# weihaoysgs/ssvio

Hardware: AMD Instinct MI355X
Metric: stereo frames/s (ORB extract + row-band match + triangulate + one local BA per frame) on 1241x376 (higher is better)
Workload: dtype u8 (front-end) + f64 (BA)

## Files before the change

### include/ssx_test_hooks.h

```cpp
#ifndef SSX_TEST_HOOKS_H
#define SSX_TEST_HOOKS_H
#include "ssx.h"

#ifdef __cplusplus
extern "C" {
#endif

SSX_API int32_t ssx_ba_window_selftest(uint32_t seed, int32_t steps);

SSX_API int64_t ssx_debug_kernel_dynamic_lds(const char* kernel);
SSX_API void ssx_debug_set_dense_slabs(int32_t mode);

SSX_API void ssx_debug_set_trial_finish(int32_t mode);

SSX_API double ssx_ba_debug_prepare_seconds(const ssx_ba_problem* prob, int32_t reps);

SSX_API int32_t ssx_ba_debug_upload_format(const ssx_ba_problem* prob);

SSX_API uint64_t ssx_ba_debug_prepare_digest(const ssx_ba_problem* prob, int32_t threads);


SSX_API ssx_status ssx_ba_linearize(ssx_ctx* ctx, const ssx_ba_problem* prob, double huber_delta, int32_t jac_mode,
                            double* Hpp, double* bp, double* Hll, double* bl, double* Hpl, double* err,
                            double* chi2);

SSX_API ssx_status ssx_orb_stage_level(ssx_ctx* ctx, int32_t image, int32_t level, int32_t blurred,
                                       uint8_t* out, int32_t out_cap, int32_t* rows, int32_t* cols);
SSX_API ssx_status ssx_orb_stage_candidates(ssx_ctx* ctx, int32_t image, int32_t level, int32_t cap,
                                            ssx_keypoint* out, int32_t* n);

SSX_API ssx_status ssx_lk_stage_level(ssx_ctx* ctx, int32_t which, int32_t level, uint8_t* out, int32_t out_cap,
                                      int32_t* rows, int32_t* cols);
SSX_API ssx_status ssx_lk_stage_deriv(ssx_ctx* ctx, int32_t level, int16_t* out, int32_t out_cap, int32_t* rows,
                                      int32_t* cols);

#ifdef __cplusplus
}
#endif
#endif
```

### ssvio_amd/csrc/octree.hip

```cpp
#include "orb_ws.hpp"

namespace ssxorb {

namespace {

typedef unsigned long long u64;
constexpr int T = OCT_THREADS;
constexpr int NW = T / 64;
constexpr unsigned NONE = 0xFFFFu;
struct Box { int16_t ulx, uly, brx, bry; };

struct Tab {
  u64* c4;
  u64* kid4;
  Box* box;
  uint32_t* key;
  uint16_t* cnt;
  uint16_t* pidx;
  uint16_t* newpos;
  uint16_t* proc;
  uint16_t* exp;
};

__device__ __forceinline__ Tab carve(uint8_t* base, int LN)
{
  Tab o;
  const size_t n = (size_t)LN;
  o.c4 = (u64*)base;
  o.kid4 = o.c4 + n;
  o.box = (Box*)(o.kid4 + n);
  o.key = (uint32_t*)(o.box + 2 * n);
  o.cnt = (uint16_t*)(o.key + n);
  o.pidx = o.cnt + 2 * n;
  o.newpos = o.pidx + n;
  o.proc = o.newpos + n;
  o.exp = o.proc + n;
  return o;
}
static_assert(OCT_NODE_BYTES == 8 + 8 + 16 + 4 + 4 + 2 + 2 + 2 + 4, "Tab layout and OCT_NODE_BYTES disagree");

__device__ __forceinline__ u64 block_scan(u64 v, u64 (*s_w)[NW], int& par, u64& total)
{
  const int lane = threadIdx.x & 63, wave = threadIdx.x >> 6;
  u64 inc = v;
#pragma unroll
  for (int o = 1; o < 64; o <<= 1) {
    const u64 up = __shfl_up(inc, o);
    if (lane >= o) inc += up;
  }
  if (lane == 63) s_w[par][wave] = inc;
  __syncthreads();
  u64 before = 0, tot = 0;
#pragma unroll
  for (int w = 0; w < NW; ++w) {
    const u64 x = s_w[par][w];
    tot += x;
    if (w < wave) before += x;
  }
  par ^= 1;
  total = tot;
  return before + (inc - v);
}

__device__ __forceinline__ int quadrant(int x, int y, const Box& n)
{
  const int mx = n.ulx + ((n.brx - n.ulx + 1) >> 1);
  const int my = n.uly + ((n.bry - n.uly + 1) >> 1);
  return (x < mx) ? ((y < my) ? 0 : 2) : ((y < my) ? 1 : 3);
}

__device__ __forceinline__ unsigned f16(u64 v, int q) { return (unsigned)((v >> (16 * q)) & 0xFFFFu); }
__device__ __forceinline__ int pk_x(uint32_t p) { return (int)(p & 0xFFF); }
__device__ __forceinline__ int pk_y(uint32_t p) { return (int)((p >> 12) & 0xFFF); }
__device__ __forceinline__ uint32_t pk_r(uint32_t p) { return p >> 24; }
__device__ __forceinline__ int nonzero4(u64 c) { return (f16(c, 0) > 0) + (f16(c, 1) > 0) + (f16(c, 2) > 0) + (f16(c, 3) > 0); }
__device__ __forceinline__ int above1_4(u64 c) { return (f16(c, 0) > 1) + (f16(c, 1) > 1) + (f16(c, 2) > 1) + (f16(c, 3) > 1); }

template <bool GLOBAL_TAB, bool GLOBAL_KEYS>
__global__ __launch_bounds__(OCT_THREADS) void k_octree(OrbDev d)
{
  extern __shared__ __attribute__((aligned(16))) uint8_t smem[];
  __shared__ u64 s_w[2][NW];
  __shared__ int s_root[64], s_rootpos[64];
  __shared__ int s_i[2];
  const int img = blockIdx.x, level = blockIdx.y, t = threadIdx.x;
  const int lane = t & 63;
  if (d.detect_only && level > 0) return;
  const int il = img * d.nlevels + level;
  const int LN = d.oct_ln;
  Tab tb;
  uint32_t* s_cellpos;
  const int CAP = d.oct_cand_cap;
  uint8_t* scratch = d.oct + (size_t)il * d.oct_stride;
  if constexpr (GLOBAL_TAB) {
    tb = carve(scratch + (GLOBAL_KEYS ? 6 * (size_t)CAP : 0), LN);
    s_cellpos = reinterpret_cast<uint32_t*>(smem);
  } else {
    tb = carve(smem, LN);
    s_cellpos = reinterpret_cast<uint32_t*>(smem + (((size_t)OCT_NODE_BYTES * LN + 15) & ~size_t(15)));
  }
  uint32_t* s_kpk;
  uint16_t* s_kn;
  if constexpr (GLOBAL_KEYS) {
    s_kpk = reinterpret_cast<uint32_t*>(scratch);
    s_kn = reinterpret_cast<uint16_t*>(s_kpk + CAP);
  } else {
    s_kpk = s_cellpos + ((d.oct_max_cells + 1 + 3) & ~3);
    s_kn = reinterpret_cast<uint16_t*>(s_kpk + CAP);
  }
  const int N = d.feat[level];
  const int cell0 = d.lvl_cell0[level], cell1 = d.lvl_cell0[level + 1];
  const int ncell = cell1 - cell0;
  const int* ccount = d.cell_count + (size_t)img * d.n_cells + cell0;
  const uint32_t* __restrict__ ccand = d.cell_cand + ((size_t)img * d.n_cells + cell0) * CELL_CAP;
  int par = 0;

  int M;
  {
    const int chunk = (ncell + T - 1) / T;
    const int lo = min(t * chunk, ncell), hi = min(lo + chunk, ncell);
    u64 mine = 0;
    for (int c = lo; c < hi; ++c) mine += (u64)ccount[c];
    u64 total;
    uint32_t pos = (uint32_t)block_scan(mine, s_w, par, total);
    for (int c = lo; c < hi; ++c) { s_cellpos[c] = pos; pos += (uint32_t)ccount[c]; }
    if (t == 0) {
      s_cellpos[ncell] = (uint32_t)total;
      d.lvl_ncand[il] = (int)total;
      if (total > (u64)CAP) atomicOr(&d.status[img], 1);
    }
    M = (int)min(total, (u64)CAP);
    if (t < 64) s_root[t] = 0;
  }
  __syncthreads();
  int* sel_count = d.sel_count + il;
  uint32_t* sel = d.sel + (size_t)il * SEL_CAP;
  if (M == 0) { if (t == 0) *sel_count = 0; return; }

  const int minX = EDGE_THRESHOLD - 3, minY = minX;
  const int maxX = d.lvl_cols[level] - EDGE_THRESHOLD + 3, maxY = d.lvl_rows[level] - EDGE_THRESHOLD + 3;
  const int nIni = (int)roundf((float)(maxX - minX) / (float)(maxY - minY));
  if (nIni < 1 || nIni > 64) { if (t == 0) *sel_count = 0; return; }
  const float hX = (float)(maxX - minX) / (float)nIni;
  const int kchunk = (M + T - 1) / T;
  const int p0 = min(t * kchunk, M);
  const int nk = min(kchunk, M - p0);
  {
    int c = 0, off = 0, cend = 0;
    if (nk > 0) {
      int lo = 0, hi = ncell;
      while (hi - lo > 1) { const int mid = (lo + hi) >> 1; if (s_cellpos[mid] <= (uint32_t)p0) lo = mid; else hi = mid; }
      c = lo;
      off = p0 - (int)s_cellpos[c];
      cend = (int)(s_cellpos[c + 1] - s_cellpos[c]);
    }
    int run_root = -1, run_n = 0;
    for (int k = 0; k < nk; ++k) {
      while (off >= cend) { ++c; off = 0; cend = (int)(s_cellpos[c + 1] - s_cellpos[c]); }
      const uint32_t v = ccand[(size_t)c * CELL_CAP + off];
      ++off;
      s_kpk[k * T + t] = v;
      const int rt = (int)((float)pk_x(v) / hX);
      const int root = rt >= nIni ? nIni - 1 : rt;
      s_kn[k * T + t] = (uint16_t)root;
      if (root != run_root) {
        if (run_n > 0) atomicAdd(&s_root[run_root], run_n);
        run_root = root; run_n = 0;
      }
      ++run_n;
    }
    if (run_n > 0) atomicAdd(&s_root[run_root], run_n);
  }
  __syncthreads();
  if (t < 64) {
    const int c = t < nIni ? s_root[t] : 0;
    const u64 bal = __ballot(c > 0);
    const int pos = __popcll(bal & ((1ull << lane) - 1ull));
    s_rootpos[t] = pos;
    if (c > 0) {
      Box b;
      b.ulx = (int16_t)(int)(hX * (float)t); b.uly = 0;
      b.brx = (int16_t)(int)(hX * (float)(t + 1)); b.bry = (int16_t)(maxY - minY);
      tb.box[pos] = b;
      tb.cnt[pos] = (uint16_t)c;
    }
    if (t == 0) s_i[0] = __popcll(bal);
  }
  __syncthreads();
  int nNodes = s_i[0];
  for (int k = 0; k < nk; ++k) s_kn[k * T + t] = (uint16_t)s_rootpos[s_kn[k * T + t]];

  int cur = 0, ecur = 0, nExp = 0, phase = 1, guard = 0;
  bool finish = false;
  while (!finish && ++guard < 256) {
    const Box* bx = tb.box + cur * LN;
    const uint16_t* ct = tb.cnt + cur * LN;
    Box* nbx = tb.box + (cur ^ 1) * LN;
    uint16_t* nct = tb.cnt + (cur ^ 1) * LN;
    const uint16_t* exp_cur = tb.exp + ecur * LN;
    uint16_t* exp_nxt = tb.exp + (ecur ^ 1) * LN;
    const int prevSize = nNodes;
    const int nchunk = (nNodes + T - 1) / T;
    const int nlo = min(t * nchunk, nNodes), nhi = min(nlo + nchunk, nNodes);
    int m = 0;
    if (phase == 1) {
      u64 mine = 0;
      for (int j = nlo; j < nhi; ++j) mine += ct[j] > 1;
      u64 total;
      uint32_t pos = (uint32_t)block_scan(mine, s_w, par, total);
      for (int j = nlo; j < nhi; ++j) {
        if (ct[j] > 1) { tb.proc[pos] = (uint16_t)j; tb.pidx[j] = (uint16_t)pos; tb.c4[pos] = 0; ++pos; }
// ... 81 lines not shown
    for (int i = plo; i < phi; ++i) {
      const int j = tb.proc[i];
      const Box x = bx[j];
      const u64 c = tb.c4[i];
      const int cc = nonzero4(c);
      const int mx = x.ulx + ((x.brx - x.ulx + 1) >> 1);
      const int my = x.uly + ((x.bry - x.uly + 1) >> 1);
      const int first = (int)Tchild - (int)run_cc - cc;
      int above = cc;
      u64 kid = 0;
      for (int q = 0; q < 4; ++q) {
        const int n = (int)f16(c, q);
        if (n == 0) continue;
        --above;
        const int id = first + above;
        Box ch;
        ch.ulx = (int16_t)((q & 1) ? mx : x.ulx); ch.brx = (int16_t)((q & 1) ? x.brx : mx);
        ch.uly = (int16_t)((q & 2) ? my : x.uly); ch.bry = (int16_t)((q & 2) ? x.bry : my);
        nbx[id] = ch;
        nct[id] = (uint16_t)n;
        kid |= (u64)id << (16 * q);
        if (n > 1) exp_nxt[run_ex++] = (uint16_t)id;
      }
      tb.kid4[i] = kid;
      run_cc += (uint32_t)cc;
    }
    for (int j = nlo; j < nhi; ++j)
      if (tb.pidx[j] == NONE) {
        const uint32_t np = Tchild + run_k++;
        tb.newpos[j] = (uint16_t)np;
        nbx[np] = bx[j];
        nct[np] = ct[j];
      }
    __syncthreads();
    for (int k = 0; k < nk; ++k) {
      const int kn = s_kn[k * T + t];
      const int j = kn & 0x3FFF, q = kn >> 14;
      const unsigned pi = tb.pidx[j];
      s_kn[k * T + t] = (pi != NONE) ? (uint16_t)f16(tb.kid4[pi], q) : tb.newpos[j];
    }
    __syncthreads();
    cur ^= 1;
    ecur ^= 1;
    nNodes = nNew;
    nExp = (int)EXtot;
    if (nNodes >= N || nNodes == prevSize) finish = true;
    else if (phase == 1 && nNodes + 3 * nExp > N) phase = 2;
  }
  __syncthreads();
  {
    uint32_t* best = tb.key;
    for (int j = t; j < nNodes; j += T) best[j] = 0;
    __syncthreads();
    {
      int run_j = -1;
      uint32_t run_best = 0;
      for (int k = 0; k < nk; ++k) {
        const int j = s_kn[k * T + t] & 0x3FFF;
        const uint32_t v = (pk_r(s_kpk[k * T + t]) << 16) | (uint32_t)(0xFFFF - (p0 + k));
        if (j != run_j) {
          if (run_j >= 0) atomicMax(&best[run_j], run_best);
          run_j = j; run_best = 0;
        }
        run_best = max(run_best, v);
      }
      if (run_j >= 0) atomicMax(&best[run_j], run_best);
    }
    __syncthreads();
    const int nOut = min(nNodes, SEL_CAP);
    for (int k = 0; k < nk; ++k) {
      const int j = s_kn[k * T + t] & 0x3FFF;
      const uint32_t c = s_kpk[k * T + t];
      if (j < nOut && best[j] == ((pk_r(c) << 16) | (uint32_t)(0xFFFF - (p0 + k)))) sel[j] = c;
    }
    if (t == 0) {
      *sel_count = nOut;
      if (nNodes > SEL_CAP) atomicOr(&d.status[img], 4);
    }
  }
}

}

void launch_octree(const OrbDev& o, hipStream_t s)
{
  const dim3 grid(o.I, o.detect_only ? 1 : o.nlevels);
  const size_t tab = o.oct_global_tab ? 0 : (((size_t)OCT_NODE_BYTES * o.oct_ln + 15) & ~size_t(15));
  const size_t lds = tab + 4 * (size_t)((o.oct_max_cells + 1 + 3) & ~3) + (o.oct_global_keys ? 0 : 6 * (size_t)o.oct_cand_cap);
  void (*kern)(OrbDev) = o.oct_global_tab ? (o.oct_global_keys ? k_octree<true, true> : k_octree<true, false>)
                                          : (o.oct_global_keys ? k_octree<false, true> : k_octree<false, false>);
  if (lds > 48 * 1024)
    (void)hipFuncSetAttribute(reinterpret_cast<const void*>(kern), hipFuncAttributeMaxDynamicSharedMemorySize, (int)lds);
  hipLaunchKernelGGL(kern, grid, dim3(OCT_THREADS), lds, s, o);
}

}
```

### ssvio_amd/csrc/orb.hip

```cpp
#include <algorithm>
#include <cfloat>
#include <cmath>
#include <vector>

#include "ctx.hpp"
#include "orb_ws.hpp"
#include "../../include/ssx_test_hooks.h"

namespace ssxorb {

__constant__ __attribute__((aligned(16))) int8_t c_pattern[256 * 4] = {
#include "brief_pattern.inc"
};
__constant__ int c_umax[16] = {15, 15, 15, 15, 14, 14, 14, 13, 13, 12, 11, 10, 9, 8, 6, 3};
__constant__ int c_gauss[7] = {18, 34, 49, 55, 49, 34, 18};
__constant__ int c_ring_dx[16] = {0, 1, 2, 3, 3, 3, 2, 1, 0, -1, -2, -3, -3, -3, -2, -1};
__constant__ int c_ring_dy[16] = {3, 3, 2, 1, 0, -1, -2, -3, -3, -3, -2, -1, 0, 1, 2, 3};

struct ResizeQuad {
  uint32_t s0;
  uint32_t sel0, sel1;
  uint32_t pad;
  uint32_t w[4];
};

constexpr int RS_ROWS = 4;
constexpr int RS_LOOP = 4;
template <bool WIDE8>
__global__ __launch_bounds__(256) void k_resize(const uint8_t* __restrict__ src_base, uint8_t* __restrict__ dst_base,
                                                size_t img_stride_bytes, int spitch, int drows, int dcols, int dpitch,
                                                const ResizeQuad* __restrict__ xtab, const uint2* __restrict__ ytab, int loops)
{
  const int q = blockIdx.x * 64 + threadIdx.x;
  if (4 * q >= dcols) return;
  const uint8_t* src = src_base + (size_t)blockIdx.z * img_stride_bytes;
  uint8_t* dst = dst_base + (size_t)blockIdx.z * img_stride_bytes;
  const uint4 ta = reinterpret_cast<const uint4*>(xtab)[2 * q], tw = reinterpret_cast<const uint4*>(xtab)[2 * q + 1];
#pragma unroll 1
  for (int it = 0; it < loops; ++it) {
  const int dy0 = ((blockIdx.y * loops + it) * 4 + __builtin_amdgcn_readfirstlane(threadIdx.y)) * RS_ROWS;
  if (dy0 >= drows) break;
  uint32_t p00[RS_ROWS], p01[RS_ROWS], p10[RS_ROWS], p11[RS_ROWS];
  int b0[RS_ROWS], b1[RS_ROWS];
  uint2 w0[RS_ROWS], w1[RS_ROWS];
#pragma unroll
  for (int r = 0; r < RS_ROWS; ++r) {
    const uint2 yt = ytab[min(dy0 + r, drows - 1)];
    b0[r] = (int)(yt.y & 0xFFFFu); b1[r] = (int)(yt.y >> 16);
    const uint8_t* r0 = src + (size_t)(yt.x & 0xFFFFu) * spitch + ta.x;
    const uint8_t* r1 = src + (size_t)(yt.x >> 16) * spitch + ta.x;
    if (WIDE8) {
      __builtin_memcpy(&w0[r], r0, 8);
      __builtin_memcpy(&w1[r], r1, 8);
    } else {
      p00[r] = p01[r] = p10[r] = p11[r] = 0;
#pragma unroll
      for (int k = 0; k < 4; ++k) {
        const int o0 = (ta.y >> (8 * k)) & 0xFF, o1 = (ta.z >> (8 * k)) & 0xFF;
        p00[r] |= (uint32_t)r0[o0] << (8 * k); p01[r] |= (uint32_t)r0[o1] << (8 * k);
        p10[r] |= (uint32_t)r1[o0] << (8 * k); p11[r] |= (uint32_t)r1[o1] << (8 * k);
      }
    }
  }
  const uint32_t wa[4] = {tw.x, tw.y, tw.z, tw.w};
#pragma unroll
  for (int r = 0; r < RS_ROWS; ++r) {
    if (WIDE8) {
      p00[r] = __builtin_amdgcn_perm(w0[r].y, w0[r].x, ta.y); p01[r] = __builtin_amdgcn_perm(w0[r].y, w0[r].x, ta.z);
      p10[r] = __builtin_amdgcn_perm(w1[r].y, w1[r].x, ta.y); p11[r] = __builtin_amdgcn_perm(w1[r].y, w1[r].x, ta.z);
    }
    uint32_t out = 0;
#pragma unroll
    for (int k = 0; k < 4; ++k) {
      const int a0 = (int)(wa[k] & 0xFFFFu), a1 = (int)(wa[k] >> 16);
      const int S0 = (int)((p00[r] >> (8 * k)) & 0xFF) * a0 + (int)((p01[r] >> (8 * k)) & 0xFF) * a1;
      const int S1 = (int)((p10[r] >> (8 * k)) & 0xFF) * a0 + (int)((p11[r] >> (8 * k)) & 0xFF) * a1;
      const uint32_t v = (uint32_t)((((b0[r] * (S0 >> 4)) >> 16) + ((b1[r] * (S1 >> 4)) >> 16) + 2) >> 2);
      out |= (v & 0xFFu) << (8 * k);
    }
    if (dy0 + r < drows) *reinterpret_cast<uint32_t*>(dst + (size_t)(dy0 + r) * dpitch + 4 * q) = out;
  }
  }
}
// ... 836 lines not shown
    for (int j = 0; j < nCols; ++j) {
      const float iniX = (float)(minBorderX + j * wCell);
      float maxX = iniX + wCell + 6;
      if (iniX >= maxBorderX - 6) continue;
      if (maxX > maxBorderX) maxX = (float)maxBorderX;
      Cell c;
      c.x0 = (int16_t)(int)iniX; c.y0 = (int16_t)(int)iniY;
      c.w = (int16_t)((int)maxX - (int)iniX); c.h = (int16_t)((int)maxY - (int)iniY);
      c.ox = (int16_t)(j * wCell); c.oy = (int16_t)(i * hCell);
      c.level = (int16_t)level; c.pad = 0;
      out.push_back(c);
    }
  }
}

}

ssx_status plan(ssx_ctx* ctx, int rows, int cols, int I, const ssx_orb_params& prm, bool has_mask, bool detect_only)
{
  OrbWorkspace* ws = get_ws(ctx);
  const int nlevels = detect_only ? 1 : prm.nlevels;
  if (rows <= 2 * EDGE_THRESHOLD || cols <= 2 * EDGE_THRESHOLD || rows > 4000 || cols > 4000) {
    ctx->set_error("ssx_orb: image %dx%d outside the supported range (40..4000 per side)", cols, rows);
    return SSX_ERR_INVALID_ARG;
  }
  if (nlevels < 1 || nlevels > MAX_LEVELS || !(prm.scale_factor > 1.0f) || prm.nfeatures < 1 || prm.nfeatures > SEL_CAP - 8 || I < 1) {
    ctx->set_error("ssx_orb: unsupported parameters (nlevels=%d scale=%g nfeatures=%d)", prm.nlevels, (double)prm.scale_factor, prm.nfeatures);
    return SSX_ERR_INVALID_ARG;
  }
  if (ws->planned && ws->rows == rows && ws->cols == cols && ws->I == I && ws->nlevels == nlevels &&
      ws->nfeatures == prm.nfeatures && ws->ini_th == prm.ini_th_fast && ws->min_th == prm.min_th_fast &&
      ws->has_mask == (int)has_mask && ws->detect_only == (int)detect_only && ws->scale_factor == prm.scale_factor)
    return SSX_OK;
  SSX_HIP_TRY(ctx, hipSetDevice(ctx->device));
  SSX_HIP_TRY(ctx, hipStreamSynchronize(ctx->stream));
  OrbDev d{};
  d.I = I; d.nlevels = nlevels; d.ini_th = prm.ini_th_fast; d.min_th = prm.min_th_fast;
  d.has_mask = has_mask; d.detect_only = detect_only;
  float scale[MAX_LEVELS], inv[MAX_LEVELS];
  scale[0] = 1.0f;
  for (int i = 1; i < nlevels; ++i) scale[i] = scale[i - 1] * prm.scale_factor;
  for (int i = 0; i < nlevels; ++i) inv[i] = 1.0f / scale[i];
  if (detect_only) {
    d.feat[0] = prm.nfeatures;
  } else {
    const float factor = 1.0f / prm.scale_factor;
    float nDesired = prm.nfeatures * (1 - factor) / (1 - (float)std::pow((double)factor, (double)nlevels));
    int sum = 0;
    for (int l = 0; l < nlevels - 1; ++l) {
      d.feat[l] = h_round(nDesired);
      sum += d.feat[l];
      nDesired *= factor;
    }
    d.feat[nlevels - 1] = std::max(prm.nfeatures - sum, 0);
  }
  std::vector<Cell> cells;
  size_t off = 0;
  int out_cap = 32;
  for (int l = 0; l < nlevels; ++l) {
    d.scale[l] = scale[l];
    d.lvl_cols[l] = h_round((float)cols * inv[l]);
    d.lvl_rows[l] = h_round((float)rows * inv[l]);
    d.lvl_pitch[l] = (d.lvl_cols[l] + 127) & ~127;
    d.lvl_off[l] = off;
    off += (size_t)d.lvl_pitch[l] * d.lvl_rows[l];
    d.lvl_cell0[l] = (int)cells.size();
    make_cells(d.lvl_rows[l], d.lvl_cols[l], l, cells);
    {
      const int bw = d.lvl_cols[l] - 2 * (EDGE_THRESHOLD - 3), bh = d.lvl_rows[l] - 2 * (EDGE_THRESHOLD - 3);
      const int n_ini = bh > 0 ? (int)std::lround((double)bw / (double)bh) : 0;
      out_cap += std::max(d.feat[l] + 4, 4 * std::max(n_ini, 0) + 4);
    }
    if (d.feat[l] + 8 > SEL_CAP) {
      ctx->set_error("ssx_orb: %d features on level %d exceed the octree node capacity", d.feat[l], l);
      return SSX_ERR_UNSUPPORTED;
    }
  }
  d.lvl_cell0[nlevels] = (int)cells.size();
  for (int l = nlevels + 1; l <= MAX_LEVELS; ++l) d.lvl_cell0[l] = (int)cells.size();
  d.n_cells = (int)cells.size();
  d.pyr_bytes = (off + 255) & ~size_t(255);
  d.out_cap = out_cap;
  {
    int maxN = 256;
    for (int l = 0; l < (detect_only ? 1 : nlevels); ++l) maxN = std::max(maxN, d.feat[l]);
    d.oct_ln = (maxN + 8 + 7) & ~7;
    d.oct_max_cells = 1;
    for (int l = 0; l < nlevels; ++l) d.oct_max_cells = std::max(d.oct_max_cells, d.lvl_cell0[l + 1] - d.lvl_cell0[l]);
    d.oct_global_keys = (size_t)d.lvl_rows[0] * d.lvl_cols[0] > 600000;
    d.oct_cand_cap = d.oct_global_keys ? CAND_CAP_BIG : CAND_CAP;
    const size_t key_lds = d.oct_global_keys ? 0 : 6 * (size_t)CAND_CAP;
    if (4 * (size_t)(d.oct_max_cells + 8) + key_lds > (size_t)OCT_LDS_BUDGET) {
      ctx->set_error("ssx_orb: %d grid cells on one level exceed the octree workgroup's LDS", d.oct_max_cells);
      return SSX_ERR_UNSUPPORTED;
    }
    d.oct_global_tab = (size_t)OCT_NODE_BYTES * d.oct_ln + 4 * (size_t)(d.oct_max_cells + 8) + key_lds > (size_t)OCT_LDS_BUDGET;
    d.oct_stride = ((d.oct_global_keys ? 6 * (size_t)CAND_CAP_BIG : 0) + (d.oct_global_tab ? (size_t)OCT_NODE_BYTES * d.oct_ln : 0) + 255) & ~size_t(255);
    if (!d.oct_global_keys && !d.oct_global_tab) d.oct_stride = 0;
  }
  {
    int tile = 16, npx = 1, t0 = 0;
    for (const Cell& c : cells) {
      const int tw = ((c.x0 & 3) + c.w + 3) & ~3;
      tile = std::max(tile, tw * (int)c.h);
      npx = std::max(npx, std::max(c.w - 6, 0) * std::max(c.h - 6, 0));
    }
    d.fast_tile_bytes = (tile + 15) & ~15;
    d.fast_lds_per_wave = 2 * d.fast_tile_bytes + ((2 * npx + 15) & ~15);
    d.gauss_run = I > 8 ? GT_RUN : 1;
    for (int l = 0; l < nlevels; ++l) {
      d.gauss_tile0[l] = t0;
      t0 += ((((d.lvl_cols[l] + GT_W - 1) / GT_W) + d.gauss_run - 1) / d.gauss_run) * ((d.lvl_rows[l] + GT_H - 1) / GT_H);
    }
    for (int l = nlevels; l <= MAX_LEVELS; ++l) d.gauss_tile0[l] = t0;
  }
  std::vector<ResizeQuad> xtab;
  std::vector<uint2> ytab;
  for (int l = 1; l < nlevels; ++l) {
    const int scols = d.lvl_cols[l - 1], srows = d.lvl_rows[l - 1], dcols = d.lvl_cols[l], drows = d.lvl_rows[l];
    const double scale_x = 1. / ((double)dcols / scols), scale_y = 1. / ((double)drows / srows);
    d.rs_xoff[l] = (int)xtab.size();
    d.rs_yoff[l] = (int)ytab.size();
    d.rs_wide8[l] = 1;
    for (int q = 0; 4 * q < dcols; ++q) {
      ResizeQuad rq{};
      for (int k = 0; k < 4 && 4 * q + k < dcols; ++k) {
        const int dx = 4 * q + k;
        float fx = (float)((dx + 0.5) * scale_x - 0.5);
        int sx = (int)std::floor(fx);
        fx -= sx;
        if (sx < 0) { fx = 0; sx = 0; }
        if (sx >= scols - 1) { fx = 0; sx = scols - 1; }
        const int a0 = h_round((1.f - fx) * 2048), a1 = h_round(fx * 2048);
        const int sx1 = std::min(sx + 1, scols - 1);
        if (k == 0) rq.s0 = (uint32_t)sx;
        const int o0 = sx - (int)rq.s0, o1 = sx1 - (int)rq.s0;
        if (o1 > 7) d.rs_wide8[l] = 0;
        if (o1 > 255) {
          ctx->set_error("ssx_orb: pyramid scale factor %g is too large for the resize tables", (double)prm.scale_factor);
          return SSX_ERR_UNSUPPORTED;
        }
        rq.sel0 |= (uint32_t)o0 << (8 * k);
        rq.sel1 |= (uint32_t)o1 << (8 * k);
        rq.w[k] = (uint32_t)a0 | ((uint32_t)a1 << 16);
      }
      xtab.push_back(rq);
    }
    for (int dy = 0; dy < drows; ++dy) {
      float fy = (float)((dy + 0.5) * scale_y - 0.5);
      const int sy = (int)std::floor(fy);
      fy -= sy;
      const int b0 = h_round((1.f - fy) * 2048), b1 = h_round(fy * 2048);
      const int sy0 = std::min(std::max(sy, 0), srows - 1), sy1 = std::min(std::max(sy + 1, 0), srows - 1);
      ytab.push_back(make_uint2((uint32_t)sy0 | ((uint32_t)sy1 << 16), (uint32_t)b0 | ((uint32_t)b1 << 16)));
    }
  }
  for (const Cell& c : cells)
    if (c.w > ROI_MAX || c.h > ROI_MAX) {
      ctx->set_error("ssx_orb: grid cell %dx%d exceeds the %d-px LDS tile", c.w, c.h, ROI_MAX);
      return SSX_ERR_UNSUPPORTED;
    }
  Layout lay;
  const size_t o_cells = lay.take(sizeof(Cell) * std::max<size_t>(cells.size(), 1));
  const size_t o_xtab = lay.take(sizeof(ResizeQuad) * std::max<size_t>(xtab.size(), 1));
  const size_t o_ytab = lay.take(sizeof(uint2) * std::max<size_t>(ytab.size(), 4));
  const size_t o_pyr = lay.take(d.pyr_bytes * I);
  const size_t o_mask = lay.take(has_mask ? d.pyr_bytes * I : 256);
  const size_t o_blur = lay.take(d.pyr_bytes * I);
  const size_t o_ccount = lay.take(sizeof(int) * (size_t)I * std::max(d.n_cells, 1));
  const size_t o_ccand = lay.take(sizeof(uint32_t) * (size_t)I * std::max(d.n_cells, 1) * CELL_CAP);
  const size_t o_oct = lay.take(std::max<size_t>(d.oct_stride * (size_t)I * nlevels, 256));
  const size_t o_ncand = lay.take(sizeof(int) * (size_t)I * nlevels);
  const size_t o_selc = lay.take(sizeof(int) * (size_t)I * nlevels);
  const size_t o_sel = lay.take(sizeof(uint32_t) * (size_t)I * nlevels * SEL_CAP);
  const size_t o_ang = lay.take(sizeof(float) * (size_t)I * nlevels * SEL_CAP);
  const size_t o_status = lay.take(sizeof(int) * (size_t)I);
  const size_t o_kps = lay.take(sizeof(ssx_keypoint) * (size_t)I * out_cap);
  const size_t o_desc = lay.take((size_t)32 * I * out_cap);
  const size_t o_n = lay.take(sizeof(int) * (size_t)I);
  SSX_HIP_TRY(ctx, ws->arena.reserve(lay.off));
  char* base = ws->arena.as<char>();
  d.cells = (const Cell*)(base + o_cells);
  d.rs_xtab = (const ResizeQuad*)(base + o_xtab);
  d.rs_ytab = (const uint2*)(base + o_ytab);
  d.pyr = (uint8_t*)(base + o_pyr);
  d.maskpyr = (uint8_t*)(base + o_mask);
  d.blur = (uint8_t*)(base + o_blur);
  d.cell_count = (int*)(base + o_ccount);
  d.cell_cand = (uint32_t*)(base + o_ccand);
  d.oct = (uint8_t*)(base + o_oct);
  d.lvl_ncand = (int*)(base + o_ncand);
  d.sel_count = (int*)(base + o_selc);
  d.sel = (uint32_t*)(base + o_sel);
  d.sel_angle = (float*)(base + o_ang);
  d.status = (int*)(base + o_status);
  d.out_kps = (uint8_t*)(base + o_kps);
  d.out_desc = (uint8_t*)(base + o_desc);
  d.out_n = (int*)(base + o_n);
  if (!cells.empty())
    SSX_HIP_TRY(ctx, hipMemcpyAsync(base + o_cells, cells.data(), sizeof(Cell) * cells.size(), hipMemcpyHostToDevice, ctx->stream));
  if (!xtab.empty()) {
    SSX_HIP_TRY(ctx, hipMemcpyAsync(base + o_xtab, xtab.data(), sizeof(ResizeQuad) * xtab.size(), hipMemcpyHostToDevice, ctx->stream));
    SSX_HIP_TRY(ctx, hipMemcpyAsync(base + o_ytab, ytab.data(), sizeof(uint2) * ytab.size(), hipMemcpyHostToDevice, ctx->stream));
  }
  SSX_HIP_TRY(ctx, hipStreamSynchronize(ctx->stream));
  ws->dev = d;
  ws->rows = rows; ws->cols = cols; ws->I = I; ws->nlevels = nlevels; ws->nfeatures = prm.nfeatures;
  ws->ini_th = prm.ini_th_fast; ws->min_th = prm.min_th_fast; ws->has_mask = has_mask; ws->detect_only = detect_only;
  ws->scale_factor = prm.scale_factor;
  ws->planned = true;
  return SSX_OK;
}

static void launch_pyramid(ssx_ctx* ctx, const OrbDev& d, hipStream_t s, int images)
{
  for (int l = 1; l < d.nlevels; ++l) {
    if (d.lvl_cols[l] <= 0 || d.lvl_rows[l] <= 0) break;
    const int loops = images > 8 ? RS_LOOP : 1;
    const dim3 grid((d.lvl_cols[l] + 255) / 256, (d.lvl_rows[l] + 4 * RS_ROWS * loops - 1) / (4 * RS_ROWS * loops), images);
    auto kern = d.rs_wide8[l] ? k_resize<true> : k_resize<false>;
    for (int m = 0; m < (d.has_mask ? 2 : 1); ++m) {
      uint8_t* pyr = m ? d.maskpyr : d.pyr;
      SSX_PROF(ctx, KID_ORB_RESIZE, hipLaunchKernelGGL(kern, grid, dim3(64, 4), 0, s, pyr + d.lvl_off[l - 1], pyr + d.lvl_off[l], d.pyr_bytes,
                         d.lvl_pitch[l - 1], d.lvl_rows[l], d.lvl_cols[l], d.lvl_pitch[l], d.rs_xtab + d.rs_xoff[l], d.rs_ytab + d.rs_yoff[l], loops));
    }
  }
}

ssx_status stage_level0(ssx_ctx* ctx, const uint8_t* imgs_dev, int stride, size_t img_bytes, const uint8_t* masks_dev,
                        int mask_stride, size_t mask_bytes)
{
  OrbWorkspace* ws = get_ws(ctx);
  const OrbDev& d = ws->dev;
  const dim3 grid((d.lvl_cols[0] + 511) / 512, (d.lvl_rows[0] + 3) / 4, d.I);
  SSX_PROF(ctx, KID_ORB_MISC, hipLaunchKernelGGL(k_copy_level0, grid, dim3(64, 4), 0, ctx->stream, imgs_dev, stride, img_bytes, d.pyr, d.pyr_bytes,
                     d.lvl_rows[0], d.lvl_cols[0], d.lvl_pitch[0]));
  if (d.has_mask)
    SSX_PROF(ctx, KID_ORB_MISC, hipLaunchKernelGGL(k_copy_level0, grid, dim3(64, 4), 0, ctx->stream, masks_dev, mask_stride, mask_bytes, d.maskpyr,
                       d.pyr_bytes, d.lvl_rows[0], d.lvl_cols[0], d.lvl_pitch[0]));
  SSX_HIP_TRY(ctx, hipGetLastError());
  return SSX_OK;
}

ssx_status run_pipeline(ssx_ctx* ctx)
{
  OrbWorkspace* ws = get_ws(ctx);
  const OrbDev& d = ws->dev;
  hipStream_t s = ctx->stream;
  SSX_HIP_TRY(ctx, hipMemsetAsync(d.status, 0, sizeof(int) * d.I, s));
  constexpr int FAST_WPW = 2;
  if (FAST_WPW * (size_t)d.fast_lds_per_wave > 48 * 1024)
    (void)hipFuncSetAttribute(reinterpret_cast<const void*>(k_fast_cells), hipFuncAttributeMaxDynamicSharedMemorySize,
                              (int)(FAST_WPW * (size_t)d.fast_lds_per_wave));
  auto launch_fast = [&](hipStream_t st, int c0, int c1) {
    if (c1 > c0)
      SSX_PROF_ON(ctx, st, KID_ORB_FAST, hipLaunchKernelGGL(k_fast_cells, dim3((c1 - c0 + FAST_WPW - 1) / FAST_WPW, d.I), dim3(64 * FAST_WPW),
                                                            FAST_WPW * (size_t)d.fast_lds_per_wave, st, d, c0, c1));
  };
  static const bool no_fork_env = getenv("SSX_ORB_NO_FORK") != nullptr;
  const bool fork = !d.detect_only && ctx->aux != nullptr && d.I > 2 && !no_fork_env;
  if (fork) {
    SSX_HIP_TRY(ctx, hipEventRecord(ctx->ev_fork, s));
    SSX_HIP_TRY(ctx, hipStreamWaitEvent(ctx->aux, ctx->ev_fork, 0));
    launch_fast(ctx->aux, 0, d.lvl_cell0[1]);
    SSX_HIP_TRY(ctx, hipEventRecord(ctx->ev_fast0, ctx->aux));
    launch_pyramid(ctx, d, s, d.I);
    SSX_HIP_TRY(ctx, hipEventRecord(ctx->ev_pyr, s));
    SSX_HIP_TRY(ctx, hipStreamWaitEvent(ctx->aux, ctx->ev_pyr, 0));
    SSX_PROF_ON(ctx, ctx->aux, KID_ORB_GAUSS, hipLaunchKernelGGL(k_gauss7, dim3(d.gauss_tile0[d.nlevels], d.I), dim3(256), 0, ctx->aux, d));
    SSX_HIP_TRY(ctx, hipEventRecord(ctx->ev_join, ctx->aux));
    launch_fast(s, d.lvl_cell0[1], d.n_cells);
    SSX_HIP_TRY(ctx, hipStreamWaitEvent(s, ctx->ev_fast0, 0));
  } else {
    launch_pyramid(ctx, d, s, d.I);
    if (!d.detect_only)
      SSX_PROF(ctx, KID_ORB_GAUSS, hipLaunchKernelGGL(k_gauss7, dim3(d.gauss_tile0[d.nlevels], d.I), dim3(256), 0, s, d));
    launch_fast(s, 0, d.n_cells);
  }
  SSX_PROF(ctx, KID_ORB_OCTREE, launch_octree(d, s));
  if (d.detect_only) {
    SSX_PROF(ctx, KID_ORB_MISC, hipLaunchKernelGGL(k_finalize_detect, dim3((SEL_CAP + 255) / 256, d.I), dim3(256), 0, s, d));
  } else {
    const dim3 kgrid((d.out_cap + 4 + 4 * OB_KPW - 1) / (4 * OB_KPW), d.I);
    if (fork) SSX_HIP_TRY(ctx, hipStreamWaitEvent(s, ctx->ev_join, 0));
    SSX_PROF(ctx, KID_ORB_BRIEF, hipLaunchKernelGGL(k_orient_brief, kgrid, dim3(256), 0, s, d));
  }
  SSX_PROF(ctx, KID_ORB_MISC, hipLaunchKernelGGL(k_counts, dim3((d.I + 63) / 64), dim3(64), 0, s, d));
  SSX_HIP_TRY(ctx, hipGetLastError());
  return SSX_OK;
}

namespace {

ssx_status run_host_image(ssx_ctx* ctx, const uint8_t* img, int stride, int rows, int cols, const uint8_t* mask,
                          int mask_stride, const ssx_orb_params& prm, bool detect_only)
{
  ssx_status st = plan(ctx, rows, cols, 1, prm, mask != nullptr, detect_only);
  if (st != SSX_OK) return st;
  OrbWorkspace* ws = get_ws(ctx);
  const size_t bytes = (size_t)rows * cols;
  SSX_HIP_TRY(ctx, ws->input.reserve(2 * bytes + 512));
  SSX_HIP_TRY(ctx, ws->stage.reserve(2 * bytes + 512));
  uint8_t* hs = ws->stage.as<uint8_t>();
  for (int y = 0; y < rows; ++y) memcpy(hs + (size_t)y * cols, img + (size_t)y * stride, cols);
  if (mask)
    for (int y = 0; y < rows; ++y) memcpy(hs + bytes + (size_t)y * cols, mask + (size_t)y * mask_stride, cols);
  SSX_HIP_TRY(ctx, hipMemcpyAsync(ws->input.p, hs, mask ? 2 * bytes : bytes, hipMemcpyHostToDevice, ctx->stream));
  st = stage_level0(ctx, ws->input.as<uint8_t>(), cols, bytes, ws->input.as<uint8_t>() + bytes, cols, bytes);
  if (st != SSX_OK) return st;
  return run_pipeline(ctx);
}

ssx_status fetch_image_result(ssx_ctx* ctx, int image, int cap, ssx_keypoint* kps_out, uint8_t* desc_out, int32_t* n)
{
  OrbWorkspace* ws = get_ws(ctx);
  const OrbDev& d = ws->dev;
  int hn[2] = {0, 0};
  SSX_HIP_TRY(ctx, hipMemcpyAsync(&hn[0], d.out_n + image, sizeof(int), hipMemcpyDeviceToHost, ctx->stream));
  SSX_HIP_TRY(ctx, hipMemcpyAsync(&hn[1], d.status + image, sizeof(int), hipMemcpyDeviceToHost, ctx->stream));
  SSX_HIP_TRY(ctx, hipStreamSynchronize(ctx->stream));
  if (hn[1] != 0) {
    ctx->set_error("ssx_orb: internal capacity exceeded (status bits %d: 1=candidates 2=octree nodes 4=outputs)", hn[1]);
    return SSX_ERR_CAPACITY;
  }
  *n = hn[0];
  if (hn[0] > cap) {
    ctx->set_error("ssx_orb: %d keypoints but capacity %d", hn[0], cap);
    return SSX_ERR_CAPACITY;
  }
  if (hn[0] > 0) {
    if (kps_out)
      SSX_HIP_TRY(ctx, hipMemcpyAsync(kps_out, d.out_kps + (size_t)image * d.out_cap * sizeof(ssx_keypoint),
                                      sizeof(ssx_keypoint) * hn[0], hipMemcpyDeviceToHost, ctx->stream));
    if (desc_out && !d.detect_only)
      SSX_HIP_TRY(ctx, hipMemcpyAsync(desc_out, d.out_desc + (size_t)image * d.out_cap * 32, (size_t)32 * hn[0],
                                      hipMemcpyDeviceToHost, ctx->stream));
    SSX_HIP_TRY(ctx, hipStreamSynchronize(ctx->stream));
  }
  return SSX_OK;
}

}

ssx_status fetch_image(ssx_ctx* ctx, int image, int cap, ssx_keypoint* kps_out, uint8_t* desc_out, int32_t* n)
{
  return fetch_image_result(ctx, image, cap, kps_out, desc_out, n);
}

}

using namespace ssxorb;

extern "C" {

void ssx_orb_default_params(ssx_orb_params* p)
{
  if (!p) return;
  p->nfeatures = 2000; p->scale_factor = 1.2f; p->nlevels = 8; p->ini_th_fast = 20; p->min_th_fast = 7;
}

ssx_status ssx_orb_detect(ssx_ctx* ctx, const uint8_t* img, int32_t stride, int32_t rows, int32_t cols,
                          const uint8_t* mask, int32_t mask_stride, const ssx_orb_params* prm, int32_t cap,
// ... 183 lines not shown
  const size_t o_desc = lay.take((size_t)32 * n_in);
  const size_t o_keep = lay.take((size_t)n_in);
  SSX_HIP_TRY(ctx, ws->input.reserve(lay.off));
  SSX_HIP_TRY(ctx, ws->stage.reserve(lay.off));
  char* hs = ws->stage.as<char>();
  for (int y = 0; y < rows; ++y) memcpy(hs + o_img + (size_t)y * cols, img + (size_t)y * stride, cols);
  memcpy(hs + o_in, kps_in, sizeof(ssx_keypoint) * n_in);
  char* base = ws->input.as<char>();
  SSX_HIP_TRY(ctx, hipMemcpyAsync(base, hs, in_bytes, hipMemcpyHostToDevice, ctx->stream));
  st = stage_level0(ctx, (const uint8_t*)(base + o_img), cols, bytes, nullptr, 0, 0);
  if (st != SSX_OK) return st;
  hipStream_t s = ctx->stream;
  launch_pyramid(ctx, d, s, 1);
  SSX_PROF(ctx, KID_ORB_GAUSS, hipLaunchKernelGGL(k_gauss7, dim3(d.gauss_tile0[d.nlevels], 1), dim3(256), 0, s, d));
  DescribeAt a;
  a.in = (const ssx_keypoint*)(base + o_in); a.out = (ssx_keypoint*)(base + o_out); a.desc = (uint8_t*)(base + o_desc);
  a.keep = (uint8_t*)(base + o_keep); a.n_in = n_in;
  SSX_PROF(ctx, KID_ORB_BRIEF, hipLaunchKernelGGL(k_describe_at, dim3((n_in + 3) / 4), dim3(256), 0, s, d, a));
  SSX_HIP_TRY(ctx, hipGetLastError());
  SSX_HIP_TRY(ctx, hipMemcpyAsync(hs + o_out, base + o_out, lay.off - o_out, hipMemcpyDeviceToHost, s));
  SSX_HIP_TRY(ctx, hipStreamSynchronize(s));
  const ssx_keypoint* ok = (const ssx_keypoint*)(hs + o_out);
  const uint8_t* od = (const uint8_t*)(hs + o_desc);
  const uint8_t* keep = (const uint8_t*)(hs + o_keep);
  int m = 0;
  for (int i = 0; i < n_in; ++i) {
    if (!keep[i]) continue;
    if (kps_out) kps_out[m] = ok[i];
    if (desc_out) memcpy(desc_out + (size_t)32 * m, od + (size_t)32 * i, 32);
    ++m;
  }
  *n = m;
  return SSX_OK;
}

#ifndef SSX_NO_TEST_HOOKS
ssx_status ssx_orb_stage_level(ssx_ctx* ctx, int32_t image, int32_t level, int32_t blurred, uint8_t* out,
                               int32_t out_cap, int32_t* rows, int32_t* cols)
{
  if (!ctx || !ctx->orb || !ctx->orb->planned) return SSX_ERR_INVALID_ARG;
  const OrbDev& d = ctx->orb->dev;
  if (image < 0 || image >= d.I || level < 0 || level >= d.nlevels) return SSX_ERR_INVALID_ARG;
  const int r = d.lvl_rows[level], c = d.lvl_cols[level];
  if (rows) *rows = r;
  if (cols) *cols = c;
  if (!out) return SSX_OK;
  if (out_cap < r * c) return SSX_ERR_CAPACITY;
  const uint8_t* src = (blurred ? d.blur : d.pyr) + (size_t)image * d.pyr_bytes + d.lvl_off[level];
  SSX_HIP_TRY(ctx, hipMemcpy2DAsync(out, c, src, d.lvl_pitch[level], c, r, hipMemcpyDeviceToHost, ctx->stream));
  SSX_HIP_TRY(ctx, hipStreamSynchronize(ctx->stream));
  return SSX_OK;
}

ssx_status ssx_orb_stage_candidates(ssx_ctx* ctx, int32_t image, int32_t level, int32_t cap, ssx_keypoint* out,
                                    int32_t* n)
{
  if (!ctx || !ctx->orb || !ctx->orb->planned || !n) return SSX_ERR_INVALID_ARG;
  const OrbDev& d = ctx->orb->dev;
  if (image < 0 || image >= d.I || level < 0 || level >= d.nlevels) return SSX_ERR_INVALID_ARG;
  const int c0 = d.lvl_cell0[level], c1 = d.lvl_cell0[level + 1];
  const int nc = c1 - c0;
  std::vector<int> cnt(std::max(nc, 1));
  std::vector<uint32_t> cand((size_t)std::max(nc, 1) * CELL_CAP);
  if (nc > 0) {
    SSX_HIP_TRY(ctx, hipMemcpyAsync(cnt.data(), d.cell_count + (size_t)image * d.n_cells + c0, sizeof(int) * nc, hipMemcpyDeviceToHost, ctx->stream));
    SSX_HIP_TRY(ctx, hipMemcpyAsync(cand.data(), d.cell_cand + ((size_t)image * d.n_cells + c0) * CELL_CAP,
                                    sizeof(uint32_t) * (size_t)nc * CELL_CAP, hipMemcpyDeviceToHost, ctx->stream));
    SSX_HIP_TRY(ctx, hipStreamSynchronize(ctx->stream));
  }
  int m = 0;
  for (int c = 0; c < nc; ++c)
    for (int k = 0; k < cnt[c]; ++k, ++m) {
      if (m >= cap || !out) continue;
      const uint32_t p = cand[(size_t)c * CELL_CAP + k];
      ssx_keypoint kp;
      kp.x = (float)(p & 0xFFF); kp.y = (float)((p >> 12) & 0xFFF); kp.size = 7.f; kp.angle = -1.f;
      kp.response = (float)(p >> 24); kp.octave = 0; kp.class_id = -1;
      out[m] = kp;
    }
  *n = m;
  return (out && m > cap) ? SSX_ERR_CAPACITY : SSX_OK;
}

#endif

}
```

### ssvio_amd/csrc/orb_ws.hpp

```cpp
#pragma once
#include <hip/hip_runtime.h>

#include <cstdint>
#include <vector>

#include "ctx.hpp"

namespace ssxorb {

constexpr int MAX_LEVELS = 8;
constexpr int CELL_CAP = 256;
constexpr int CAND_CAP = 16384;
constexpr int CAND_CAP_BIG = 65536;
constexpr int SEL_CAP = 4096;
constexpr int EDGE_THRESHOLD = 19;
constexpr int OCT_THREADS = 1024;

struct Cell {
  int16_t x0, y0;
  int16_t w, h;
  int16_t ox, oy;
  int16_t level, pad;
};

constexpr int OCT_NODE_BYTES = 50;
constexpr int OCT_LDS_BUDGET = 158 * 1024;

struct ResizeQuad;

struct OrbDev {
  int I;
  int nlevels;
  int lvl_rows[MAX_LEVELS], lvl_cols[MAX_LEVELS], lvl_pitch[MAX_LEVELS];
  size_t lvl_off[MAX_LEVELS];
  size_t pyr_bytes;
  float scale[MAX_LEVELS];
  int feat[MAX_LEVELS];
  int lvl_cell0[MAX_LEVELS + 1];
  int n_cells;
  int ini_th, min_th;
  int has_mask;
  int detect_only;
  int out_cap;
  int fast_tile_bytes;
  int fast_lds_per_wave;
  int gauss_tile0[MAX_LEVELS + 1];
  int gauss_run;
  int rs_xoff[MAX_LEVELS], rs_yoff[MAX_LEVELS];
  int rs_wide8[MAX_LEVELS];
  const Cell* cells;
  const ResizeQuad* rs_xtab;
  const uint2* rs_ytab;
  uint8_t* pyr;
  uint8_t* maskpyr;
  uint8_t* blur;
  int* cell_count;
  uint32_t* cell_cand;
  uint8_t* oct;
  size_t oct_stride;
  int oct_max_cells;
  int oct_cand_cap;
  int oct_global_keys;
  int oct_ln;
  int oct_global_tab;
  int* lvl_ncand;
  int* sel_count;
  uint32_t* sel;
  float* sel_angle;
  int* status;
  uint8_t* out_kps;
  uint8_t* out_desc;
  int* out_n;
};

void launch_octree(const OrbDev& o, hipStream_t s);

}

struct OrbWorkspace {
  DevBuf arena;
  DevBuf input;
  DevBuf stereo;
  HostBuf stage;
  HostBuf fetch;
  ssxorb::OrbDev dev{};
  int rows = 0, cols = 0, I = 0, nlevels = 0, nfeatures = 0, ini_th = 0, min_th = 0, has_mask = 0, detect_only = 0;
  float scale_factor = 0.f;
  bool planned = false;
  const uint8_t* batch_imgs = nullptr;
  int batch_pairs = 0, batch_stride = 0;
  ssx_orb_params batch_orb{};
  ssx_match_params batch_mp{};
  ssx_stereo_rig batch_rig{};
  int* match_idx = nullptr;
  int* match_dist = nullptr;
  double* xyz = nullptr;
  uint8_t* tri_ok = nullptr;
  int* pair_counts = nullptr;
  DevBuf ingest[2];
  hipStream_t copy_stream = nullptr;
  hipEvent_t ev_up[2] = {nullptr, nullptr}, ev_free[2] = {nullptr, nullptr};
  bool free_pending[2] = {false, false};
  int up_first = 0, up_count = 0;
  int up_shape[2][4] = {{0, 0, 0, 0}, {0, 0, 0, 0}};
  HostBuf counts_pinned;
  hipEvent_t ev_counts[2] = {nullptr, nullptr};
  int cnt_first = 0, cnt_count = 0, cnt_pairs[2] = {0, 0};
  ssx_status cnt_fail[2] = {SSX_OK, SSX_OK};
};

namespace ssxorb {
OrbWorkspace* get_ws(ssx_ctx* ctx);
ssx_status plan(ssx_ctx* ctx, int rows, int cols, int I, const ssx_orb_params& prm, bool has_mask, bool detect_only);
ssx_status run_pipeline(ssx_ctx* ctx);
ssx_status fetch_image(ssx_ctx* ctx, int image, int cap, ssx_keypoint* kps_out, uint8_t* desc_out, int32_t* n);
ssx_status stage_level0(ssx_ctx* ctx, const uint8_t* imgs_dev, int stride, size_t img_bytes, const uint8_t* masks_dev,
                        int mask_stride, size_t mask_bytes);
}
```

Measured before the change: 17920.

## Size octree kernel block per level from candidate count via rung ladder

```diff
diff --git a/include/ssx_test_hooks.h b/include/ssx_test_hooks.h
--- a/include/ssx_test_hooks.h
+++ b/include/ssx_test_hooks.h
@@ -29,6 +29,10 @@
 SSX_API ssx_status ssx_orb_stage_candidates(ssx_ctx* ctx, int32_t image, int32_t level, int32_t cap,
                                             ssx_keypoint* out, int32_t* n);
 
+SSX_API void ssx_debug_set_octree_rung(int32_t rung);
+SSX_API int32_t ssx_debug_octree_rung_threads(int32_t rung);
+SSX_API ssx_status ssx_orb_stage_octree_rungs(ssx_ctx* ctx, int32_t image, int32_t cap, int32_t* rung, int32_t* ncand, int32_t* n);
+
 SSX_API ssx_status ssx_lk_stage_level(ssx_ctx* ctx, int32_t which, int32_t level, uint8_t* out, int32_t out_cap,
                                       int32_t* rows, int32_t* cols);
 SSX_API ssx_status ssx_lk_stage_deriv(ssx_ctx* ctx, int32_t level, int16_t* out, int32_t out_cap, int32_t* rows,
diff --git a/ssvio_amd/csrc/octree.hip b/ssvio_amd/csrc/octree.hip
--- a/ssvio_amd/csrc/octree.hip
+++ b/ssvio_amd/csrc/octree.hip
@@ -1,3 +1,5 @@
+#include <algorithm>
+
 #include "orb_ws.hpp"
 
 namespace ssxorb {
@@ -5,8 +7,6 @@
 namespace {
 
 typedef unsigned long long u64;
-constexpr int T = OCT_THREADS;
-constexpr int NW = T / 64;
 constexpr unsigned NONE = 0xFFFFu;
 struct Box { int16_t ulx, uly, brx, bry; };
 
@@ -39,6 +39,7 @@
 }
 static_assert(OCT_NODE_BYTES == 8 + 8 + 16 + 4 + 4 + 2 + 2 + 2 + 4, "Tab layout and OCT_NODE_BYTES disagree");
 
+template <int NW>
 __device__ __forceinline__ u64 block_scan(u64 v, u64 (*s_w)[NW], int& par, u64& total)
 {
   const int lane = threadIdx.x & 63, wave = threadIdx.x >> 6;
@@ -76,9 +77,35 @@
 __device__ __forceinline__ int nonzero4(u64 c) { return (f16(c, 0) > 0) + (f16(c, 1) > 0) + (f16(c, 2) > 0) + (f16(c, 3) > 0); }
 __device__ __forceinline__ int above1_4(u64 c) { return (f16(c, 0) > 1) + (f16(c, 1) > 1) + (f16(c, 2) > 1) + (f16(c, 3) > 1); }
 
-template <bool GLOBAL_TAB, bool GLOBAL_KEYS>
-__global__ __launch_bounds__(OCT_THREADS) void k_octree(OrbDev d)
-{
+__device__ __forceinline__ int rung_for(unsigned total, int min_rung)
+{
+  int r = 0;
+#pragma unroll
+  for (int i = 0; i < OCT_RUNGS - 1; ++i) r += total > (unsigned)oct_rung_cap(i);
+  return max(r, min_rung);
+}
+
+__global__ __launch_bounds__(256) void k_octree_plan(OrbDev d)
+{
+  const int nlv = d.detect_only ? 1 : d.nlevels;
+  const int w = blockIdx.x * 4 + (threadIdx.x >> 6), lane = threadIdx.x & 63;
+  if (w >= d.I * nlv) return;
+  const int img = w / nlv, level = w - img * nlv;
+  const int cell0 = d.lvl_cell0[level], ncell = d.lvl_cell0[level + 1] - cell0;
+  const int* ccount = d.cell_count + (size_t)img * d.n_cells + cell0;
+  unsigned sum = 0;
+  for (int c = lane; c < ncell; c += 64) sum += (unsigned)ccount[c];
+#pragma unroll
+  for (int o = 32; o > 0; o >>= 1) sum += __shfl_xor(sum, o);
+  if (lane == 0) d.lvl_rung[img * d.nlevels + level] = rung_for(sum, d.oct_min_rung);
+}
+
+template <int RUNG, bool GLOBAL_TAB, bool GLOBAL_KEYS>
+__global__ __launch_bounds__(oct_rung_threads(RUNG)) void k_octree(OrbDev d)
+{
+  constexpr int T = oct_rung_threads(RUNG), NW = T / 64;
+  constexpr bool LADDER = !GLOBAL_TAB && !GLOBAL_KEYS;
+  static_assert(LADDER || RUNG == OCT_RUNGS - 1, "the global-scratch variants run on the last rung");
   extern __shared__ __attribute__((aligned(16))) uint8_t smem[];
   __shared__ u64 s_w[2][NW];
   __shared__ int s_root[64], s_rootpos[64];
@@ -87,10 +114,12 @@
   const int lane = t & 63;
   if (d.detect_only && level > 0) return;
   const int il = img * d.nlevels + level;
-  const int LN = d.oct_ln;
+  if constexpr (LADDER)
+    if (d.lvl_rung[il] != RUNG) return;
+  const int LN = d.oct_lvl_ln[level];
   Tab tb;
   uint32_t* s_cellpos;
-  const int CAP = d.oct_cand_cap;
+  const int CAP = GLOBAL_KEYS ? d.oct_cand_cap : oct_rung_cap(RUNG);
   uint8_t* scratch = d.oct + (size_t)il * d.oct_stride;
   if constexpr (GLOBAL_TAB) {
     tb = carve(scratch + (GLOBAL_KEYS ? 6 * (size_t)CAP : 0), LN);
@@ -127,6 +156,7 @@
     if (t == 0) {
       s_cellpos[ncell] = (uint32_t)total;
       d.lvl_ncand[il] = (int)total;
+      if constexpr (!LADDER) d.lvl_rung[il] = RUNG;
       if (total > (u64)CAP) atomicOr(&d.status[img], 1);
     }
     M = (int)min(total, (u64)CAP);
@@ -374,16 +404,45 @@
 
 }
 
-void launch_octree(const OrbDev& o, hipStream_t s)
-{
-  const dim3 grid(o.I, o.detect_only ? 1 : o.nlevels);
+namespace {
+
+template <int RUNG>
+void launch_rung(const OrbDev& o, const dim3& grid, size_t lds_fixed, hipStream_t s)
+{
+  const size_t lds = lds_fixed + 6 * (size_t)oct_rung_cap(RUNG);
+  if (lds > 48 * 1024)
+    (void)hipFuncSetAttribute(reinterpret_cast<const void*>(k_octree<RUNG, false, false>), hipFuncAttributeMaxDynamicSharedMemorySize, (int)lds);
+  hipLaunchKernelGGL((k_octree<RUNG, false, false>), grid, dim3(oct_rung_threads(RUNG)), lds, s, o);
+}
+
+}
+
+void launch_octree(const OrbDev& dev, hipStream_t s, int min_rung)
+{
+  OrbDev o = dev;
+  const int nlv = o.detect_only ? 1 : o.nlevels;
+  const dim3 grid(o.I, nlv);
   const size_t tab = o.oct_global_tab ? 0 : (((size_t)OCT_NODE_BYTES * o.oct_ln + 15) & ~size_t(15));
-  const size_t lds = tab + 4 * (size_t)((o.oct_max_cells + 1 + 3) & ~3) + (o.oct_global_keys ? 0 : 6 * (size_t)o.oct_cand_cap);
-  void (*kern)(OrbDev) = o.oct_global_tab ? (o.oct_global_keys ? k_octree<true, true> : k_octree<true, false>)
-                                          : (o.oct_global_keys ? k_octree<false, true> : k_octree<false, false>);
-  if (lds > 48 * 1024)
-    (void)hipFuncSetAttribute(reinterpret_cast<const void*>(kern), hipFuncAttributeMaxDynamicSharedMemorySize, (int)lds);
-  hipLaunchKernelGGL(kern, grid, dim3(OCT_THREADS), lds, s, o);
-}
-
-}
+  const size_t lds_fixed = tab + 4 * (size_t)((o.oct_max_cells + 1 + 3) & ~3);
+  constexpr int LAST = OCT_RUNGS - 1;
+  if (o.oct_global_tab || o.oct_global_keys) {
+    o.oct_min_rung = LAST;
+    const size_t lds = lds_fixed + (o.oct_global_keys ? 0 : 6 * (size_t)o.oct_cand_cap);
+    void (*kern)(OrbDev) = o.oct_global_tab ? (o.oct_global_keys ? k_octree<LAST, true, true> : k_octree<LAST, true, false>)
+                                            : k_octree<LAST, false, true>;
+    if (lds > 48 * 1024)
+      (void)hipFuncSetAttribute(reinterpret_cast<const void*>(kern), hipFuncAttributeMaxDynamicSharedMemorySize, (int)lds);
+    hipLaunchKernelGGL(kern, grid, dim3(oct_rung_threads(LAST)), lds, s, o);
+    return;
+  }
+  o.oct_min_rung = std::min(std::max(min_rung, 0), LAST);
+  hipLaunchKernelGGL(k_octree_plan, dim3((o.I * nlv + 3) / 4), dim3(256), 0, s, o);
+  launch_rung<4>(o, grid, lds_fixed, s);
+  launch_rung<3>(o, grid, lds_fixed, s);
+  launch_rung<2>(o, grid, lds_fixed, s);
+  launch_rung<1>(o, grid, lds_fixed, s);
+  launch_rung<0>(o, grid, lds_fixed, s);
+  static_assert(OCT_RUNGS == 5, "launch_octree names every rung");
+}
+
+}
diff --git a/ssvio_amd/csrc/orb.hip b/ssvio_amd/csrc/orb.hip
--- a/ssvio_amd/csrc/orb.hip
+++ b/ssvio_amd/csrc/orb.hip
@@ -1,4 +1,5 @@
 #include <algorithm>
+#include <atomic>
 #include <cfloat>
 #include <cmath>
 #include <vector>
@@ -1001,9 +1002,12 @@
   d.pyr_bytes = (off + 255) & ~size_t(255);
   d.out_cap = out_cap;
   {
-    int maxN = 256;
-    for (int l = 0; l < (detect_only ? 1 : nlevels); ++l) maxN = std::max(maxN, d.feat[l]);
-    d.oct_ln = (maxN + 8 + 7) & ~7;
+    d.oct_ln = 0;
+    for (int l = 0; l < MAX_LEVELS; ++l) d.oct_lvl_ln[l] = (256 + 8 + 7) & ~7;
+    for (int l = 0; l < (detect_only ? 1 : nlevels); ++l) {
+      d.oct_lvl_ln[l] = (std::max(256, d.feat[l]) + 8 + 7) & ~7;
+      d.oct_ln = std::max(d.oct_ln, d.oct_lvl_ln[l]);
+    }
     d.oct_max_cells = 1;
     for (int l = 0; l < nlevels; ++l) d.oct_max_cells = std::max(d.oct_max_cells, d.lvl_cell0[l + 1] - d.lvl_cell0[l]);
     d.oct_global_keys = (size_t)d.lvl_rows[0] * d.lvl_cols[0] > 600000;
@@ -1090,6 +1094,7 @@
   const size_t o_ccand = lay.take(sizeof(uint32_t) * (size_t)I * std::max(d.n_cells, 1) * CELL_CAP);
   const size_t o_oct = lay.take(std::max<size_t>(d.oct_stride * (size_t)I * nlevels, 256));
   const size_t o_ncand = lay.take(sizeof(int) * (size_t)I * nlevels);
+  const size_t o_rung = lay.take(sizeof(int) * (size_t)I * nlevels);
   const size_t o_selc = lay.take(sizeof(int) * (size_t)I * nlevels);
   const size_t o_sel = lay.take(sizeof(uint32_t) * (size_t)I * nlevels * SEL_CAP);
   const size_t o_ang = lay.take(sizeof(float) * (size_t)I * nlevels * SEL_CAP);
@@ -1109,6 +1114,7 @@
   d.cell_cand = (uint32_t*)(base + o_ccand);
   d.oct = (uint8_t*)(base + o_oct);
   d.lvl_ncand = (int*)(base + o_ncand);
+  d.lvl_rung = (int*)(base + o_rung);
   d.sel_count = (int*)(base + o_selc);
   d.sel = (uint32_t*)(base + o_sel);
   d.sel_angle = (float*)(base + o_ang);
@@ -1160,6 +1166,8 @@
   SSX_HIP_TRY(ctx, hipGetLastError());
   return SSX_OK;
 }
+
+static std::atomic<int> g_oct_min_rung{0};
 
 ssx_status run_pipeline(ssx_ctx* ctx)
 {
@@ -1196,7 +1204,7 @@
       SSX_PROF(ctx, KID_ORB_GAUSS, hipLaunchKernelGGL(k_gauss7, dim3(d.gauss_tile0[d.nlevels], d.I), dim3(256), 0, s, d));
     launch_fast(s, 0, d.n_cells);
   }
-  SSX_PROF(ctx, KID_ORB_OCTREE, launch_octree(d, s));
+  SSX_PROF(ctx, KID_ORB_OCTREE, launch_octree(d, s, g_oct_min_rung.load(std::memory_order_relaxed)));
   if (d.detect_only) {
     SSX_PROF(ctx, KID_ORB_MISC, hipLaunchKernelGGL(k_finalize_detect, dim3((SEL_CAP + 255) / 256, d.I), dim3(256), 0, s, d));
   } else {
@@ -1546,6 +1554,24 @@
   return (out && m > cap) ? SSX_ERR_CAPACITY : SSX_OK;
 }
 
+void ssx_debug_set_octree_rung(int32_t rung) { ssxorb::g_oct_min_rung.store(std::min(std::max(rung, 0), OCT_RUNGS - 1)); }
+
+int32_t ssx_debug_octree_rung_threads(int32_t rung) { return rung >= 0 && rung < OCT_RUNGS ? oct_rung_threads(rung) : 0; }
+
+ssx_status ssx_orb_stage_octree_rungs(ssx_ctx* ctx, int32_t image, int32_t cap, int32_t* rung, int32_t* ncand, int32_t* n)
+{
+  if (!ctx || !ctx->orb || !ctx->orb->planned || !n) return SSX_ERR_INVALID_ARG;
+  const OrbDev& d = ctx->orb->dev;
+  if (image < 0 || image >= d.I) return SSX_ERR_INVALID_ARG;
+  const int nlv = d.detect_only ? 1 : d.nlevels;
+  *n = nlv;
+  if (cap < nlv) return SSX_ERR_CAPACITY;
+  if (rung) SSX_HIP_TRY(ctx, hipMemcpyAsync(rung, d.lvl_rung + (size_t)image * d.nlevels, sizeof(int) * nlv, hipMemcpyDeviceToHost, ctx->stream));
+  if (ncand) SSX_HIP_TRY(ctx, hipMemcpyAsync(ncand, d.lvl_ncand + (size_t)image * d.nlevels, sizeof(int) * nlv, hipMemcpyDeviceToHost, ctx->stream));
+  SSX_HIP_TRY(ctx, hipStreamSynchronize(ctx->stream));
+  return SSX_OK;
+}
+
 #endif
 
 }
diff --git a/ssvio_amd/csrc/orb_ws.hpp b/ssvio_amd/csrc/orb_ws.hpp
--- a/ssvio_amd/csrc/orb_ws.hpp
+++ b/ssvio_amd/csrc/orb_ws.hpp
@@ -14,7 +14,11 @@
 constexpr int CAND_CAP_BIG = 65536;
 constexpr int SEL_CAP = 4096;
 constexpr int EDGE_THRESHOLD = 19;
-constexpr int OCT_THREADS = 1024;
+constexpr int OCT_RUNGS = 5;
+constexpr int OCT_KEYS_PER_THREAD = 16;
+__host__ __device__ constexpr int oct_rung_threads(int r) { return r == 0 ? 128 : r == 1 ? 256 : r == 2 ? 512 : r == 3 ? 768 : 1024; }
+__host__ __device__ constexpr int oct_rung_cap(int r) { return OCT_KEYS_PER_THREAD * oct_rung_threads(r); }
+static_assert(oct_rung_cap(OCT_RUNGS - 1) == CAND_CAP, "the last rung holds CAND_CAP candidates");
 
 struct Cell {
   int16_t x0, y0;
@@ -61,9 +65,12 @@
   int oct_max_cells;
   int oct_cand_cap;
   int oct_global_keys;
+  int oct_lvl_ln[MAX_LEVELS];
   int oct_ln;
   int oct_global_tab;
+  int oct_min_rung;
   int* lvl_ncand;
+  int* lvl_rung;
   int* sel_count;
   uint32_t* sel;
   float* sel_angle;
@@ -73,7 +80,7 @@
   int* out_n;
 };
 
-void launch_octree(const OrbDev& o, hipStream_t s);
+void launch_octree(const OrbDev& o, hipStream_t s, int min_rung);
 
 }
 
```

Result: no change. 17870 (median of 2 runs) (-0.3%).
